# Griffan/FASTQuick

Hardware: AMD Instinct MI355X
Metric: paired_150bp_reads_aligned_per_sec (higher is better)
Workload: dtype u32

## Files before the change

### fastquick_amd/csrc/fq_align.cpp

```cpp
#include <algorithm>
#include <atomic>
#include <ctime>
#include <chrono>
#include <climits>
#include <cstdint>
#include <cmath>
#include <cstdio>
#include <cstdlib>
#include <cstring>
#include <memory>
#include <string>
#include <unordered_map>
#include <mutex>
#include <thread>
#include <vector>
#include <pthread.h>
#include <sched.h>

#include "../../include/fastquick_amd.h"
#include "fq_backend.h"
#include "fq_index.h"
#include "fq_pipeline.h"
#include "fq_pool.h"
#include "fq_text_batch.h"
// ... 368 lines not shown
  else if (k == "gap_long_always") c->kn.gap_long_always = (int)v;
  else if (k == "gap_pool") c->kn.gap_pool = (uint32_t)v;
  else if (k == "gap_nogap_min") c->kn.gap_nogap_min = v;
  else if (k == "gap_pipeline_min") c->kn.gap_pipeline_min = v;
  else if (k == "gap_pipeline_segs") c->kn.gap_pipeline_segs = (int)std::max<int64_t>(2, std::min<int64_t>(v, 64));
  else if (k == "gap_split_hard") c->kn.gap_split_hard = v;
  else if (k == "gap_long_pops2") c->kn.gap_long_pops2 = (uint32_t)v;
  else if (k == "gap_skip_bound") c->kn.gap_skip_bound = v;
  else if (k == "gap_no_order") c->kn.gap_no_order = (int)v;
  else if (k == "device_turns") c->kn.device_turns = (int)v;
  else if (k == "device_turn_min") c->kn.device_turn_min = v;
  else if (k == "device_turn_slots") c->kn.device_turn_slots = (int)std::max<int64_t>(1, v);
  else if (k == "gap_round2_waves") c->kn.gap_round2_waves = (int)v;
  else if (k == "gap_round2_lane_major") c->kn.gap_round2_lane_major = (int)v;
  else if (k == "gap_round1_refill") c->kn.gap_round1_refill = (int)v;
  else if (k == "gap_round2_refill") c->kn.gap_round2_refill = (int)v;
  else if (k == "sw_wave_max") c->kn.sw_wave_max = (int)v;
  else if (k == "host_threads") c->kn.host_threads = (int)v;
  else if (k == "host_par_min") c->kn.host_par_min = (size_t)v;
  else if (k == "packed_bulk_min") c->kn.packed_bulk_min = v;
  else if (k == "md_mask_min") c->kn.md_mask_min = v;
  else if (k == "trace") c->kn.trace = (int)v;
  else if (k == "gap_order_asc") t->gap_order_asc = (int)v;
  else if (k == "gap_waves_per_cu") t->gap_waves_per_cu = (int)v;
  else if (k == "gap_coop_waves") t->gap_coop_waves = (int)v;
  else if (k == "gap_refill_min") t->gap_refill_min = (int)v;
  else if (k == "filter_no_turns") t->filter_no_turns = (int)v;
  else if (k == "prep_priority") t->prep_priority = (int)v;
  else if (k == "refine_lanes") t->refine_lanes = (int)v;
  else if (k == "gap_generic_opts") t->gap_generic_opts = (int)v;
  else if (k == "sw_serial_reverse") t->sw_serial_reverse = (int)v;
  else if (k == "width_both_strands") t->width_both_strands = (int)v;
  else if (k == "spin_sync") t->spin_sync = (int)v;
  else return FQ_EINVAL;
  return FQ_OK;
}

extern "C" void fq_stats_get(const fq_ctx_t *c, fq_stats_t *out) { if (c && out) *out = c->stats; }
extern "C" void fq_stats_reset(fq_ctx_t *c) { if (c) memset(&c->stats, 0, sizeof c->stats); }

#define CK(expr)                                                  \
  do {                                                            \
    if ((expr)) { c->err = std::string(#expr) + ": " + fqdev::last_error(); return FQ_ENODEV; } \
  } while (0)
#define CKM(expr)                                                 \
  do {                                                            \
    if (!(expr)) { c->err = std::string("out of device memory: ") + #expr; return FQ_ENOMEM; } \
  } while (0)

static int h2d_staged(fq_ctx *c, void *dst, const void *src, size_t bytes) {
  if (!bytes) return 0;
  void *p = c->arena.alloc(bytes);
  if (!p) { c->err = "out of pinned host memory"; return FQ_ENOMEM; }
  memcpy(p, src, bytes);
  if (fqdev::copy_pinned(dst, p, bytes, 1)) { c->err = std::string("h2d: ") + fqdev::last_error(); return FQ_ENODEV; }
  return 0;
}
static int d2h_staged(fq_ctx *c, void *dst, const void *src, size_t bytes) {
  if (!bytes) return 0;
  void *p = c->arena.alloc(bytes);
  if (!p) { c->err = "out of pinned host memory"; return FQ_ENOMEM; }
  if (fqdev::copy_pinned(p, src, bytes, 0)) { c->err = std::string("d2h: ") + fqdev::last_error(); return FQ_ENODEV; }
  c->arena.pending.push_back({dst, p, bytes});
  return 0;
}
static int sync_staged(fq_ctx *c) {
// ... 2027 lines not shown
```

### fastquick_amd/csrc/fq_backend.h

```cpp
#pragma once
#include "fq_kernels.h"
#include "fq_records.h"
#include "fq_frontend.h"
#include "fq_emit.h"
#include "fq_deflate.h"

namespace fqdev {

struct State;
struct Tune {
  int gap_coop_waves = 0;
  int gap_waves_per_cu = 0, gap_refill_min = 0, gap_order_asc = 0, filter_no_turns = 0, refine_lanes = 0;
  int spin_sync = 0;
  int gap_generic_opts = 0;
  int width_both_strands = 0;
  int prep_priority = 0;
  int sw_serial_reverse = 0;
};
int runtime_configure(int hw_queues, int blocking_waits);
int device_count();
State *state_create(int device_ordinal);
void state_destroy(State *s);
int bind(State *s);
Tune *tune(State *s);
const char *last_error();
bool is_real_gpu();
void device_turn_begin(int slots = 1);
void device_turn_end();

void *dmalloc(size_t bytes);
void dfree(void *p);
void *hmalloc(size_t bytes);
void hfree(void *p);
int h2d(void *dst, const void *src, size_t bytes);
int d2h(void *dst, const void *src, size_t bytes);
int copy_pinned(void *dst, const void *src, size_t bytes, int to_device);
int d2d(void *dst, const void *src, size_t bytes);
int dzero(void *dst, size_t bytes);
int dfill(void *dst, int byte, size_t bytes);
int sync();
int h2d_copy(void *dst, const void *src, size_t bytes);
int copy_record(int slot);
int copy_wait(int slot);
void copy_discard();
int compute_wait_copy(int slot);
int copy_flush_now();

void time_begin(int kid);
void time_end(int kid);
// ... 52 lines not shown
```

### fastquick_amd/csrc/fq_device.hip

```cpp
#include <hip/hip_runtime.h>
#include <hip/hip_ext.h>

#include <algorithm>
#include <condition_variable>
#include <atomic>
#include <cstdio>
#include <cstdlib>
#include <cstring>
#include <mutex>
#include <string>
#include <unordered_map>
#include <vector>
#include <sys/mman.h>
#include <sys/syscall.h>
#include <unistd.h>

#include "fq_backend.h"

namespace fqdev {

struct Pending { int kid; hipEvent_t a, b; };
struct State {
  int device = 0;
  hipStream_t stream = nullptr;
  hipStream_t main_stream = nullptr, aux_stream = nullptr;
  hipEvent_t fork_ev = nullptr, join_ev = nullptr;
  hipEvent_t marks[4] = {nullptr, nullptr, nullptr, nullptr};
  hipEvent_t prio_fork = nullptr;
  hipStream_t copy_stream = nullptr;
  hipEvent_t copy_done[2] = {nullptr, nullptr};
  hipEvent_t prep_done = nullptr;
  hipEvent_t sync_ev = nullptr;
  std::vector<Pending> pending;
  std::vector<hipEvent_t> free_events;
  hipEvent_t open_begin[16] = {};
  struct SmallCopy { uint8_t *dst; const uint8_t *src; size_t bytes; };
  SmallCopy small[8];
  int n_small = 0;
  uint64_t *scan_tmp = nullptr; size_t scan_tmp_n = 0;
  uint32_t *cmp_cnt = nullptr; uint64_t *cmp_off = nullptr; size_t cmp_n = 0;
  Tune tune;
};
static thread_local State *g_cur = nullptr;
static thread_local std::string g_err;
#define g_stream (g_cur->stream)

#define FQ_HIP(call)                                                                         \
  do {                                                                                       \
    hipError_t e_ = (call);                                                                  \
    if (e_ != hipSuccess) {                                                                  \
      g_err = std::string(#call) + ": " + hipGetErrorString(e_);                             \
      return -3;                                                                             \
    }                                                                                        \
  } while (0)

int copy_flush();
#define FQ_PRE() do { if (copy_flush()) return -3; } while (0)
void copy_discard() { if (g_cur) g_cur->n_small = 0; }
int copy_flush_now() { FQ_PRE(); return 0; }

const char *last_error() { return g_err.c_str(); }
bool is_real_gpu() { return true; }

static int set_kernel_attributes();
static std::mutex g_dev_mu;
static bool g_dev_ready[64];
static hipEvent_t g_prep_last[64];
static State *g_prep_owner[64];
static hipStream_t g_copy_streams[64][2];
static unsigned g_copy_next[64];
static std::mutex g_turn_mu[64];
static std::condition_variable g_turn_cv[64];
static int g_turn_held[64];
static int g_ctx_count[64];
static hipStream_t g_prio_stream[64];
static bool g_queue_warned = false;
static int g_rt_blocking_waits = 0;
int runtime_configure(int hw_queues, int blocking_waits) {
  if (hw_queues > 0) {
    char b[16];
    snprintf(b, sizeof b, "%d", hw_queues);
    setenv("GPU_MAX_HW_QUEUES", b, 0);
  }
  g_rt_blocking_waits = blocking_waits ? 1 : 0;
  return 0;
}

int device_count() { int n = 0; if (hipGetDeviceCount(&n) != hipSuccess) { (void)hipGetLastError(); return 0; } return n < 0 ? 0 : n; }
void device_turn_begin(int slots) {
  const int d = g_cur->device;
  std::unique_lock<std::mutex> lk(g_turn_mu[d]);
// ... 48 lines not shown
  if (s->fork_ev) (void)hipEventDestroy(s->fork_ev);
  if (s->join_ev) (void)hipEventDestroy(s->join_ev);
  for (hipEvent_t m : s->marks) if (m) (void)hipEventDestroy(m);
  if (s->prio_fork) (void)hipEventDestroy(s->prio_fork);
  if (s->stream) (void)hipStreamSynchronize(s->stream);
  if (s->copy_stream) (void)hipStreamSynchronize(s->copy_stream);
  {
    std::lock_guard<std::mutex> lk(g_dev_mu);
    if (g_prep_owner[s->device] == s) { g_prep_owner[s->device] = nullptr; g_prep_last[s->device] = nullptr; }
    if (g_ctx_count[s->device] > 0) --g_ctx_count[s->device];
  }
  for (auto &p : s->pending) { (void)hipEventDestroy(p.a); (void)hipEventDestroy(p.b); }
  for (auto e : s->free_events) (void)hipEventDestroy(e);
  for (auto e : s->copy_done) if (e) (void)hipEventDestroy(e);
  if (s->prep_done) (void)hipEventDestroy(s->prep_done);
  if (s->scan_tmp) (void)hipFree(s->scan_tmp);
  if (s->cmp_cnt) (void)hipFree(s->cmp_cnt);
  if (s->cmp_off) (void)hipFree(s->cmp_off);
  if (s->stream) (void)hipStreamDestroy(s->stream);
  delete s;
}
Tune *tune(State *s) { return &s->tune; }
int bind(State *s) {
  if (!s) { g_err = "no device state"; return -3; }
  if (g_cur != s) { FQ_HIP(hipSetDevice(s->device)); g_cur = s; }
  return 0;
}

void *dmalloc(size_t bytes) {
  void *p = nullptr;
  if (hipMalloc(&p, bytes ? bytes : 16) != hipSuccess) { g_err = "hipMalloc failed (" + std::to_string(bytes) + " B)"; return nullptr; }
  return p;
}
void dfree(void *p) { if (p) (void)hipFree(p); }
static const size_t kRegisterMin = (size_t)4 << 20;
static std::mutex g_reg_mu;
static std::unordered_map<void *, size_t> g_registered;
static int device_numa_node(int dev) {
  static std::mutex mu;
  static std::unordered_map<int, int> cache;
  std::lock_guard<std::mutex> lk(mu);
  auto it = cache.find(dev);
  if (it != cache.end()) return it->second;
  int node = -1;
  char bus[64] = {0};
  if (hipDeviceGetPCIBusId(bus, (int)sizeof bus, dev) == hipSuccess) {
    for (char *c = bus; *c; ++c) if (*c >= 'A' && *c <= 'F') *c = (char)(*c - 'A' + 'a');
    const std::string path = std::string("/sys/bus/pci/devices/") + bus + "/numa_node";
    if (FILE *f = fopen(path.c_str(), "r")) { if (fscanf(f, "%d", &node) != 1) node = -1; fclose(f); }
  } else (void)hipGetLastError();
  cache[dev] = node;
  return node;
}
static void prefer_node(void *m, size_t len, int node) {
  if (node < 0 || node >= 1024) return;
  unsigned long mask[16] = {0};
  mask[node / (8 * sizeof(unsigned long))] |= 1ul << (node % (8 * sizeof(unsigned long)));
  (void)syscall(SYS_mbind, m, len, 1 , mask, (unsigned long)(8 * sizeof mask + 1), 0u);
}
void *hmalloc(size_t bytes) {
  static const bool use_register = [] { const char *e = getenv("FASTQUICK_PIN_REGISTER"); return !(e && *e == '0'); }();
  if (use_register && bytes >= kRegisterMin) {
    const size_t len = (bytes + ((size_t)2 << 20) - 1) & ~(((size_t)2 << 20) - 1);
    void *m = mmap(nullptr, len, PROT_READ | PROT_WRITE, MAP_PRIVATE | MAP_ANONYMOUS, -1, 0);
    if (m != MAP_FAILED) {
      (void)madvise(m, len, MADV_HUGEPAGE);
      int dev = 0;
      if (hipGetDevice(&dev) == hipSuccess) prefer_node(m, len, device_numa_node(dev)); else (void)hipGetLastError();
      if (hipHostRegister(m, len, hipHostRegisterDefault) == hipSuccess) {
        std::lock_guard<std::mutex> lk(g_reg_mu);
        g_registered[m] = len;
        return m;
      }
      (void)hipGetLastError();
      munmap(m, len);
    }
  }
  void *p = nullptr;
  if (hipHostMalloc(&p, bytes ? bytes : 16, hipHostMallocDefault) != hipSuccess) { g_err = "hipHostMalloc failed"; return nullptr; }
  return p;
}
void hfree(void *p) {
  if (!p) return;
  size_t len = 0;
  {
    std::lock_guard<std::mutex> lk(g_reg_mu);
    auto it = g_registered.find(p);
    if (it != g_registered.end()) { len = it->second; g_registered.erase(it); }
  }
  if (len) { (void)hipHostUnregister(p); munmap(p, len); }
  else (void)hipHostFree(p);
}
int h2d(void *dst, const void *src, size_t bytes) { FQ_PRE(); if (bytes) FQ_HIP(hipMemcpyAsync(dst, src, bytes, hipMemcpyHostToDevice, g_stream)); return 0; }
int d2h(void *dst, const void *src, size_t bytes) { FQ_PRE(); if (bytes) FQ_HIP(hipMemcpyAsync(dst, src, bytes, hipMemcpyDeviceToHost, g_stream)); return 0; }
int d2d(void *dst, const void *src, size_t bytes) { FQ_PRE(); if (bytes) FQ_HIP(hipMemcpyAsync(dst, src, bytes, hipMemcpyDeviceToDevice, g_stream)); return 0; }
int dzero(void *dst, size_t bytes) { FQ_PRE(); if (bytes) FQ_HIP(hipMemsetAsync(dst, 0, bytes, g_stream)); return 0; }
int dfill(void *dst, int byte, size_t bytes) { FQ_PRE(); if (bytes) FQ_HIP(hipMemsetAsync(dst, byte, bytes, g_stream)); return 0; }
int sync() {
  FQ_PRE();
  if (g_cur->tune.spin_sync || !g_cur->sync_ev) { FQ_HIP(hipStreamSynchronize(g_stream)); return 0; }
  FQ_HIP(hipEventRecord(g_cur->sync_ev, g_stream));
  FQ_HIP(hipEventSynchronize(g_cur->sync_ev));
  return 0;
}
int stream_aux(int on) {
  FQ_PRE();
  if (on && !g_cur->aux_stream) {
    FQ_HIP(hipStreamCreateWithFlags(&g_cur->aux_stream, hipStreamNonBlocking));
    FQ_HIP(hipEventCreateWithFlags(&g_cur->fork_ev, hipEventDisableTiming));
    FQ_HIP(hipEventCreateWithFlags(&g_cur->join_ev, hipEventDisableTiming));
  }
  g_cur->stream = on ? g_cur->aux_stream : g_cur->main_stream;
  return 0;
}
int stream_fork() {
  FQ_PRE();
  if (!g_cur->aux_stream) return 0;
  FQ_HIP(hipEventRecord(g_cur->fork_ev, g_cur->main_stream));
  FQ_HIP(hipStreamWaitEvent(g_cur->aux_stream, g_cur->fork_ev, 0));
  return 0;
}
int stream_join() {
  FQ_PRE();
  if (!g_cur->aux_stream) return 0;
  FQ_HIP(hipEventRecord(g_cur->join_ev, g_cur->aux_stream));
  FQ_HIP(hipStreamWaitEvent(g_cur->main_stream, g_cur->join_ev, 0));
  return 0;
}
int stream_mark(int k) {
  FQ_PRE();
  hipEvent_t &m = g_cur->marks[k & 3];
  if (!m) FQ_HIP(hipEventCreateWithFlags(&m, hipEventDisableTiming));
  FQ_HIP(hipEventRecord(m, g_stream));
  return 0;
}
int stream_wait_mark(int k) {
  FQ_PRE();
  hipEvent_t m = g_cur->marks[k & 3];
  if (m) FQ_HIP(hipStreamWaitEvent(g_stream, m, 0));
  return 0;
}
static int copy_stream_get() {
  if (g_cur->copy_stream) return 0;
  std::lock_guard<std::mutex> lk(g_dev_mu);
  const int dev = g_cur->device;
  for (int k = 0; k < 2; ++k)
    if (!g_copy_streams[dev][k]) FQ_HIP(hipStreamCreateWithFlags(&g_copy_streams[dev][k], hipStreamNonBlocking));
  g_cur->copy_stream = g_copy_streams[dev][g_copy_next[dev]++ & 1];
  return 0;
}
int h2d_copy(void *dst, const void *src, size_t bytes) {
  if (copy_stream_get()) return -3;
  if (bytes) FQ_HIP(hipMemcpyAsync(dst, src, bytes, hipMemcpyHostToDevice, g_cur->copy_stream));
  return 0;
}
int copy_record(int slot) { if (copy_stream_get()) return -3; FQ_HIP(hipEventRecord(g_cur->copy_done[slot & 1], g_cur->copy_stream)); return 0; }
int copy_wait(int slot) { FQ_HIP(hipEventSynchronize(g_cur->copy_done[slot & 1])); return 0; }
int compute_wait_copy(int slot) { FQ_PRE(); FQ_HIP(hipStreamWaitEvent(g_stream, g_cur->copy_done[slot & 1], 0)); return 0; }

struct FqCopySet { uint8_t *dst[8]; const uint8_t *src[8]; size_t bytes[8]; };
__global__ void __launch_bounds__(256) k_copy_bytes(FqCopySet cs) {
  uint8_t *dst = cs.dst[blockIdx.y];
  const uint8_t *src = cs.src[blockIdx.y];
  const size_t bytes = cs.bytes[blockIdx.y];
  const size_t n16 = ((((uintptr_t)dst | (uintptr_t)src) & 15) == 0) ? bytes / 16 : 0;
  const size_t t = (size_t)blockIdx.x * blockDim.x + threadIdx.x, stride = (size_t)gridDim.x * blockDim.x;
  for (size_t i = t; i < n16; i += stride) ((uint4 *)dst)[i] = ((const uint4 *)src)[i];
  for (size_t i = n16 * 16 + t; i < bytes; i += stride) dst[i] = src[i];
}
static const size_t kSmallCopy = (size_t)8 << 20;
int copy_flush() {
  State *s = g_cur;
  if (!s || s->n_small == 0) return 0;
  FqCopySet cs;
  size_t most = 0;
  for (int k = 0; k < 8; ++k) {
    const bool on = k < s->n_small;
    cs.dst[k] = on ? s->small[k].dst : nullptr; cs.src[k] = on ? s->small[k].src : nullptr; cs.bytes[k] = on ? s->small[k].bytes : 0;
    if (on) most = std::max(most, s->small[k].bytes);
  }
  const int n = s->n_small;
  s->n_small = 0;
  const unsigned blocks = (unsigned)std::min<size_t>(256, (most / 16 + 255) / 256 + 1);
  hipLaunchKernelGGL(k_copy_bytes, dim3(blocks, (unsigned)n), dim3(256), 0, s->stream, cs);
  FQ_HIP(hipGetLastError());
  return 0;
}
int copy_pinned(void *dst, const void *src, size_t bytes, int to_device) {
  if (!bytes) return 0;
  if (bytes > kSmallCopy) { FQ_PRE(); FQ_HIP(hipMemcpyAsync(dst, src, bytes, to_device ? hipMemcpyHostToDevice : hipMemcpyDeviceToHost, g_stream)); return 0; }
  if (g_cur->n_small == 8) FQ_PRE();
  g_cur->small[g_cur->n_small++] = {(uint8_t *)dst, (const uint8_t *)src, bytes};
  return 0;
}

static hipEvent_t get_event() {
  if (!g_cur->free_events.empty()) { hipEvent_t e = g_cur->free_events.back(); g_cur->free_events.pop_back(); return e; }
  hipEvent_t e;
  (void)hipEventCreate(&e);
  return e;
}
void time_begin(int kid) { (void)copy_flush(); hipEvent_t e = get_event(); (void)hipEventRecord(e, g_stream); g_cur->open_begin[kid] = e; }
void time_end(int kid) { (void)copy_flush(); hipEvent_t e = get_event(); (void)hipEventRecord(e, g_stream); g_cur->pending.push_back({kid, g_cur->open_begin[kid], e}); }
static void kernel_events(int kid, hipEvent_t *a, hipEvent_t *b) { *a = get_event(); *b = get_event(); g_cur->pending.push_back({kid, *a, *b}); }
void time_collect(double ms[], uint64_t launches[], int n_ids) {
  std::vector<decltype(g_cur->pending)::value_type> later;
  for (auto &p : g_cur->pending) {
    if (hipEventQuery(p.b) == hipErrorNotReady) { later.push_back(p); continue; }
    float t = 0.f;
    if (hipEventElapsedTime(&t, p.a, p.b) == hipSuccess && p.kid < n_ids) { ms[p.kid] += t; launches[p.kid] += 1; }
    g_cur->free_events.push_back(p.a);
    g_cur->free_events.push_back(p.b);
  }
  g_cur->pending.swap(later);
}

static inline unsigned nblk(uint64_t n, unsigned b) { return (unsigned)((n + b - 1) / b); }

__global__ void __launch_bounds__(256) k_prep(FqPrepArgs a) {
  const int r = blockIdx.x * blockDim.x + threadIdx.x;
  if (r < a.n_reads) fq_prep_thread(a, r);
}
extern __shared__ __align__(16) unsigned char fq_dyn_lds[];
__global__ void __launch_bounds__(256) k_width(FqWidthArgs a) {
  uint8_t *seed_bits = (uint8_t *)fq_dyn_lds;
  const int w = blockIdx.x * blockDim.x + threadIdx.x;
// ... 356 lines not shown
  for (uint32_t base = 0; base < nb; base += 256) {
    const uint32_t i = base + threadIdx.x;
    const uint64_t v = i < nb ? blk_tot[i] : 0;
    const int lane = threadIdx.x & 63, wid = threadIdx.x >> 6;
    __shared__ uint64_t ws[4];
    uint64_t x = v;
#pragma unroll
    for (int d = 1; d < 64; d <<= 1) {
      const uint64_t y = __shfl_up(x, d, 64);
      if (lane >= d) x += y;
    }
    if (lane == 63) ws[wid] = x;
    __syncthreads();
    uint64_t b = carry, tot = 0;
    for (int k = 0; k < 4; ++k) { if (k < wid) b += ws[k]; tot += ws[k]; }
    if (i < nb) blk_tot[i] = b + x - v;
    __syncthreads();
    if (threadIdx.x == 0) carry += tot;
    __syncthreads();
  }
  if (threadIdx.x == 0) blk_tot[nb] = carry;
}
__global__ void __launch_bounds__(256) k_scan_c(const uint32_t *in, uint32_t n, const uint64_t *blk_off, uint64_t *out) {
  const uint32_t i = blockIdx.x * 256 + threadIdx.x;
  uint32_t tot;
  const uint32_t e = block_excl_scan(i < n ? in[i] : 0u, &tot);
  if (i < n) out[i] = blk_off[blockIdx.x] + e;
  if (i == 0) out[n] = blk_off[gridDim.x];
}

#define g_scan_tmp (g_cur->scan_tmp)
#define g_scan_tmp_n (g_cur->scan_tmp_n)
int launch_scan(const uint32_t *in, uint64_t *out, uint32_t n) {
  FQ_PRE();
  if (n == 0) { uint64_t z = 0; return h2d(out, &z, 8) ? -3 : sync(); }
  const unsigned nb = nblk(n, 256);
  if (g_scan_tmp_n < nb + 1) {
    dfree(g_scan_tmp);
    g_scan_tmp_n = (size_t)nb * 2 + 64;
    g_scan_tmp = (uint64_t *)dmalloc(g_scan_tmp_n * 8);
    if (!g_scan_tmp) return -4;
  }
  hipLaunchKernelGGL(k_scan_a, dim3(nb), dim3(256), 0, g_stream, in, n, g_scan_tmp);
  hipLaunchKernelGGL(k_scan_b, dim3(1), dim3(256), 0, g_stream, g_scan_tmp, nb);
  hipLaunchKernelGGL(k_scan_c, dim3(nb), dim3(256), 0, g_stream, in, n, g_scan_tmp, out);
  FQ_HIP(hipGetLastError());
  return 0;
}

__global__ void __launch_bounds__(256) k_compact_a(const uint8_t *filt, int n_pairs, uint32_t *pair_cnt, uint32_t *read_cnt) {
  const int p = blockIdx.x * 256 + threadIdx.x;
  uint32_t keep = 0, nr = 0;
  if (p < n_pairs) {
    const uint32_t f0 = filt[p], f1 = filt[n_pairs + p];
    keep = !(f0 && f1);
    nr = (!f0) + (!f1);
  }
  const unsigned long long bal = __ballot(keep);
  __shared__ uint32_t s_pairs[4], s_reads[4];
  uint32_t x = nr;
#pragma unroll
  for (int d = 32; d >= 1; d >>= 1) x += __shfl_xor(x, d, 64);
  if ((threadIdx.x & 63) == 0) { s_pairs[threadIdx.x >> 6] = (uint32_t)__popcll(bal); s_reads[threadIdx.x >> 6] = x; }
  __syncthreads();
  if (threadIdx.x == 0) {
    pair_cnt[blockIdx.x] = s_pairs[0] + s_pairs[1] + s_pairs[2] + s_pairs[3];
// ... 8 lines not shown
  const uint32_t nr = (!f0) + (!f1);
  uint32_t tot_p, tot_r;
  const uint32_t rank_p = block_excl_scan(keep, &tot_p);
  const uint32_t rank_r = block_excl_scan(nr, &tot_r);
  if (p < n_pairs) {
    if (keep) pair_list[pair_off[blockIdx.x] + rank_p] = p;
    uint32_t s = (uint32_t)read_off[blockIdx.x] + rank_r;
    if (!f0) { read_list[s] = p; sidx[p] = (int32_t)s; ++s; } else sidx[p] = -1;
    if (!f1) { read_list[s] = n_pairs + p; sidx[n_pairs + p] = (int32_t)s; } else sidx[n_pairs + p] = -1;
  }
  if (p == 0) { counts[0] = (int32_t)read_off[gridDim.x]; counts[1] = (int32_t)pair_off[gridDim.x]; }
}
#define g_cmp_cnt (g_cur->cmp_cnt)
#define g_cmp_off (g_cur->cmp_off)
#define g_cmp_n (g_cur->cmp_n)
int launch_compact(const uint8_t *filtered, int n_pairs, int32_t *read_list, int32_t *sidx, int32_t *pair_list, int32_t *counts) {
  FQ_PRE();
  if (n_pairs <= 0) return dzero(counts, 8);
  const unsigned nb = nblk((uint64_t)n_pairs, 256);
  if (g_cmp_n < nb) {
    dfree(g_cmp_cnt); dfree(g_cmp_off);
    g_cmp_n = (size_t)nb * 2 + 64;
    g_cmp_cnt = (uint32_t *)dmalloc(g_cmp_n * 2 * 4);
    g_cmp_off = (uint64_t *)dmalloc((g_cmp_n + 2) * 2 * 8);
    if (!g_cmp_cnt || !g_cmp_off) return -4;
  }
  uint32_t *pc = g_cmp_cnt, *rc = g_cmp_cnt + g_cmp_n;
  uint64_t *po = g_cmp_off, *ro = g_cmp_off + g_cmp_n + 2;
  hipLaunchKernelGGL(k_compact_a, dim3(nb), dim3(256), 0, g_stream, filtered, n_pairs, pc, rc);
  int rc1 = launch_scan(pc, po, nb);
  if (rc1) return rc1;
  rc1 = launch_scan(rc, ro, nb);
  if (rc1) return rc1;
  hipLaunchKernelGGL(k_compact_c, dim3(nb), dim3(256), 0, g_stream, filtered, n_pairs, po, ro, read_list, sidx, pair_list, counts);
  FQ_HIP(hipGetLastError());
  return 0;
}

__global__ void __launch_bounds__(256) k_bitmap_scatter(uint8_t *bitmap, const uint32_t *bits, uint64_t n) {
  const uint64_t i = (uint64_t)blockIdx.x * blockDim.x + threadIdx.x;
  if (i >= n) return;
  const uint32_t x = bits[i];
  atomicOr((unsigned int *)(bitmap + ((x >> 5) << 2)), 1u << (x & 31));
}
int launch_bitmap_scatter(uint8_t *bitmap, const uint32_t *bits, uint64_t n) {
  FQ_PRE();
  if (!n) return 0;
  hipLaunchKernelGGL(k_bitmap_scatter, dim3(nblk(n, 256)), dim3(256), 0, g_stream, bitmap, bits, n);
  FQ_HIP(hipGetLastError());
  return 0;
}

__global__ void __launch_bounds__(256) k_bitmap_kmers(FqBitmapArgs a) {
  const int64_t idx = (int64_t)blockIdx.x * 256 + threadIdx.x;
  if (idx >= 2 * a.l_pac) return;
  fq_bitmap_kmer_thread(a, idx, [&](int t, uint32_t x) { atomicOr(&a.bitmap[t][x >> 5], 1u << (x & 31)); });
}
int launch_bitmap_kmers(const FqBitmapArgs &a) {
  FQ_PRE();
  if (a.l_pac <= 0 || a.n_rec <= 0) return 0;
  hipLaunchKernelGGL(k_bitmap_kmers, dim3(nblk((uint64_t)(2 * a.l_pac), 256)), dim3(256), 0, g_stream, a);
  FQ_HIP(hipGetLastError());
  return 0;
}

static FqzCrcConst *g_crc_const[64];
// ... 65 lines not shown
  const int lane = threadIdx.x & 63;
#pragma unroll
  for (int d = 1; d < 64; d <<= 1) { const uint32_t y = (uint32_t)__shfl_up((int)x, d, 64); if (lane >= d) x += y; }
  __shared__ uint32_t s[4];
  if (lane == 63) s[threadIdx.x >> 6] = x;
  __syncthreads();
  uint32_t base = 0;
  for (int w = 0; w < (int)(threadIdx.x >> 6); ++w) base += s[w];
  uint64_t rank = blk_off[blockIdx.x] + base + (x - c);
  while (m) {
    const int j = __ffs((int)m) - 1;
    m &= m - 1;
    if (rank < cap) nl[rank] = at + (uint32_t)j;
    ++rank;
  }
}
__global__ void __launch_bounds__(64) k_nl_total(const uint64_t *blk_off, uint32_t nb, uint32_t *count) {
  if (threadIdx.x == 0) { const uint64_t t = blk_off[nb]; *count = t > 0xffffffffull ? 0xffffffffu : (uint32_t)t; }
}
int launch_nl_index(const uint8_t *text, uint32_t n, uint32_t lo, uint32_t *nl, uint32_t cap, uint32_t *count) {
  FQ_PRE();
  const unsigned nb = nblk((uint64_t)n, 4096);
  if (nb == 0) { FQ_HIP(hipMemsetAsync(count, 0, 4, g_stream)); return 0; }
  if (g_cmp_n < (size_t)nb + 1) {
    dfree(g_cmp_cnt); dfree(g_cmp_off);
    g_cmp_n = (size_t)nb * 2 + 64;
    g_cmp_cnt = (uint32_t *)dmalloc(g_cmp_n * 2 * 4);
    g_cmp_off = (uint64_t *)dmalloc((g_cmp_n + 2) * 2 * 8);
    if (!g_cmp_cnt || !g_cmp_off) { g_cmp_n = 0; return -4; }
  }
  hipLaunchKernelGGL(k_nl_count, dim3(nb), dim3(256), 0, g_stream, text, n, lo, g_cmp_cnt);
  FQ_HIP(hipGetLastError());
  if (launch_scan(g_cmp_cnt, g_cmp_off, nb)) return -3;
  hipLaunchKernelGGL(k_nl_fill, dim3(nb), dim3(256), 0, g_stream, text, n, lo, (const uint64_t *)g_cmp_off, nl, cap);
  hipLaunchKernelGGL(k_nl_total, dim3(1), dim3(64), 0, g_stream, (const uint64_t *)g_cmp_off, nb, count);
  FQ_HIP(hipGetLastError());
  return 0;
}
__global__ void __launch_bounds__(256) k_tok_rec(FqTokArgs a) {
  const int i = blockIdx.x * 256 + threadIdx.x;
  FqTokStat t = i < a.n_rec ? fqt_rec_thread(a, i) : fqt_stat_none();
#pragma unroll
  for (int d = 32; d >= 1; d >>= 1) {
    t.first_bad = min(t.first_bad, (uint32_t)__shfl_xor((int)t.first_bad, d, 64));
    t.max_name = max(t.max_name, (uint32_t)__shfl_xor((int)t.max_name, d, 64));
    t.min_name = min(t.min_name, (uint32_t)__shfl_xor((int)t.min_name, d, 64));
    t.max_len = max(t.max_len, (uint32_t)__shfl_xor((int)t.max_len, d, 64));
    t.min_len = min(t.min_len, (uint32_t)__shfl_xor((int)t.min_len, d, 64));
  }
  if ((threadIdx.x & 63) == 0) fqt_stat_commit(a, t);
}
__global__ void __launch_bounds__(256) k_tok_pieces(FqTokArgs a, int64_t n) {
  const int64_t g = (int64_t)blockIdx.x * 256 + threadIdx.x;
  if (g < n) fqt_piece_thread(a, g);
}
__global__ void __launch_bounds__(256) k_slot_bases(FqSlotArgs a) {
  const int s = blockIdx.x * 256 + threadIdx.x;
  if (s < a.n_slots) fqt_slot_bases_thread(a, s);
}
__global__ void __launch_bounds__(256) k_slot_names(FqSlotArgs a) {
  const int s = blockIdx.x * 256 + threadIdx.x;
  if (s < a.n_slots) fqt_slot_names_thread(a, s);
}
__global__ void __launch_bounds__(256) k_text_gather(FqTextGatherArgs a, int64_t n) {
  const int64_t g = (int64_t)blockIdx.x * 256 + threadIdx.x;
  if (g < n) fqt_gather_piece(a, g);
// ... 24 lines not shown
  FQ_HIP(hipGetLastError());
  return 0;
}
__global__ void __launch_bounds__(256) k_names_plain(FqSlotArgs a) {
  const int i = blockIdx.x * 256 + threadIdx.x;
  if (i < a.n_rec) fqt_names_plain_thread(a, i);
}
int launch_slot_names(const FqSlotArgs &a) {
  FQ_PRE();
  if (a.n_rec <= 0) return 0;
  if (a.plain_names) {
    hipLaunchKernelGGL(k_names_plain, dim3(nblk((uint64_t)a.n_rec, 256)), dim3(256), 0, g_stream, a);
    if (a.mode != 0) { FQ_HIP(hipGetLastError()); return 0; }
  }
  hipLaunchKernelGGL(k_slot_names, dim3(nblk((uint64_t)a.n_slots, 256)), dim3(256), 0, g_stream, a);
  FQ_HIP(hipGetLastError());
  return 0;
}
int launch_text_gather(const FqTextGatherArgs &a) {
  FQ_PRE();
  const int64_t n = (int64_t)a.n_out * (a.stride >> 4);
  if (n <= 0) return 0;
  hipLaunchKernelGGL(k_text_gather, dim3(nblk((uint64_t)n, 256)), dim3(256), 0, g_stream, a, n);
  FQ_HIP(hipGetLastError());
  return 0;
}
int launch_text_trim_all(const FqTextTrimArgs &a) {
  FQ_PRE();
  if (a.n_rows <= 0) return 0;
  hipLaunchKernelGGL(k_text_trim_all, dim3(nblk((uint64_t)a.n_rows, 256)), dim3(256), 0, g_stream, a);
  FQ_HIP(hipGetLastError());
  return 0;
}
int dfill32(void *dst, uint32_t v, size_t n_words) { FQ_PRE(); if (n_words) FQ_HIP(hipMemsetD32Async((hipDeviceptr_t)dst, (int)v, n_words, g_stream)); return 0; }

int launch_prep(const FqPrepArgs &a) {
  FQ_PRE();
  if (a.n_reads <= 0) return 0;
  hipEvent_t e0, e1;
  kernel_events(FQ_K_PREP_KERNEL, &e0, &e1);
  if (!g_cur->tune.filter_no_turns) {
    const int dev = g_cur->device;
    std::lock_guard<std::mutex> lk(g_dev_mu);
    if (g_prep_last[dev] && g_prep_owner[dev] != g_cur) FQ_HIP(hipStreamWaitEvent(g_stream, g_prep_last[dev], 0));
    hipExtLaunchKernelGGL(k_prep, dim3(nblk((uint64_t)a.n_reads, 256)), dim3(256), 0, g_stream, e0, e1, 0, a);
    FQ_HIP(hipEventRecord(g_cur->prep_done, g_stream));
    g_prep_last[dev] = g_cur->prep_done; g_prep_owner[dev] = g_cur;
  } else {
    hipExtLaunchKernelGGL(k_prep, dim3(nblk((uint64_t)a.n_reads, 256)), dim3(256), 0, g_stream, e0, e1, 0, a);
  }
  FQ_HIP(hipGetLastError());
  return 0;
}
__global__ void __launch_bounds__(256) k_surv_gather(const int32_t *pair_list, int n_surv, int n_pairs, const int32_t *len_trim, const uint8_t *filtered, const int32_t *sidx, FqSurvInfo *out) {
  const int t = blockIdx.x * blockDim.x + threadIdx.x;
  if (t < 2 * n_surv) fq_surv_gather_thread(pair_list, n_pairs, len_trim, filtered, sidx, out, t);
}
int launch_surv_gather(const int32_t *pair_list, int n_surv, int n_pairs, const int32_t *len_trim, const uint8_t *filtered, const int32_t *sidx, FqSurvInfo *out) {
  FQ_PRE();
  if (n_surv <= 0) return 0;
  hipLaunchKernelGGL(k_surv_gather, dim3(nblk((uint64_t)n_surv * 2, 256)), dim3(256), 0, g_stream, pair_list, n_surv, n_pairs, len_trim, filtered, sidx, out);
  FQ_HIP(hipGetLastError());
  return 0;
}
__global__ void __launch_bounds__(256) k_prep_packed(FqPrepPackedArgs a) {
  const int r = blockIdx.x * blockDim.x + threadIdx.x;
  if (r < a.n_reads) fq_prep_packed_thread(a, r);
// ... 131 lines not shown
    base[threadIdx.x] = h[threadIdx.x] ? start + atomicAdd(&cnt[FQ_ORDER_KEYS + threadIdx.x], h[threadIdx.x]) : 0u;
  }
  __syncthreads();
  if (w < n) order[base[key] + rank] = w;
  if (blockIdx.x == 0 && threadIdx.x == 0) {
    uint32_t sp = 0;
    if (asc) { for (int k = 0; k < FQ_ORDER_KEYS / 2; ++k) sp += cnt[k]; }
    else { for (int k = FQ_ORDER_KEYS / 2; k < FQ_ORDER_KEYS; ++k) sp += cnt[k]; }
    cnt[2 * FQ_ORDER_KEYS] = sp;
  }
}
__global__ void __launch_bounds__(256) k_collect(const int32_t *order, const uint32_t *split, int n_work, int seg, int n_seg, const uint32_t *status, const int32_t *work,
                                                  int32_t *out, uint32_t *count) {
  const uint32_t sp = split ? *split : (uint32_t)n_work;
  const uint32_t blk_start[2] = {0u, sp}, blk_len[2] = {sp, (uint32_t)n_work - sp};
  const uint32_t t = blockIdx.x * blockDim.x + threadIdx.x, stride = gridDim.x * blockDim.x;
  for (int b = 0; b < 2; ++b) {
    uint32_t lo, hi;
    fq_seg_range(blk_len[b], seg, n_seg, &lo, &hi);
    for (uint32_t pos = blk_start[b] + lo + t; pos < blk_start[b] + hi; pos += stride) {
      const int w = order ? order[pos] : (int)pos;
      if (status[w]) out[atomicAdd(count, 1u)] = work[w];
    }
  }
}
int launch_collect(const int32_t *order, const uint32_t *split, int n_work, int seg, int n_seg, const uint32_t *status, const int32_t *work, int32_t *out, uint32_t *count) {
  FQ_PRE();
  if (n_work <= 0) return 0;
  hipLaunchKernelGGL(k_collect, dim3(1024), dim3(256), 0, g_stream, order, split, n_work, seg, n_seg, status, work, out, count);
  FQ_HIP(hipGetLastError());
  return 0;
}
int launch_order(const uint8_t *bid_end, int n, int n_hard, int32_t *order, uint32_t *cnt) {
  FQ_PRE();
  if (n <= 0) return 0;
  FQ_HIP(hipMemsetAsync(cnt, 0, (2 * FQ_ORDER_KEYS + 1) * 4, g_stream));
  hipLaunchKernelGGL(k_order_count, dim3(nblk((uint64_t)n, 256)), dim3(256), 0, g_stream, bid_end, n, n_hard, cnt);
  hipLaunchKernelGGL(k_order_scatter, dim3(nblk((uint64_t)n, 256)), dim3(256), 0, g_stream, bid_end, n, n_hard, cnt, order, g_cur->tune.gap_order_asc ? 1 : 0);
  FQ_HIP(hipGetLastError());
  return 0;
}
int gap_lane_slots(const FqGapArgs &a) {
  if (a.n_work <= 0) return 0;
  if (a.tier.coop) {
    const unsigned cw = g_cur->tune.gap_coop_waves > 0 ? (unsigned)g_cur->tune.gap_coop_waves : 1024u;
    unsigned w = std::min<unsigned>((unsigned)a.n_work, a.tier.exact ? 64u : cw);
    if (a.max_waves > 0) w = std::min<unsigned>(w, (unsigned)a.max_waves);
    return (int)w;
  }
  const int env_waves = g_cur->tune.gap_waves_per_cu;
  const unsigned need = nblk((uint64_t)a.n_work, 64);
  unsigned per_cu = 8;
  if (a.tier.pool_cap <= 65535u) {
    const size_t lds = (size_t)64 * (size_t)a.o.n_buckets * 2 + (size_t)64 * FQ_COLD_N * 4;
    per_cu = (unsigned)std::max<size_t>(1, std::min<size_t>(a.tier.nogap ? FQ_NOGAP_WAVES_PER_CU : 16, (150 * 1024) / lds));
  }
  if (env_waves > 0) per_cu = std::min<unsigned>(per_cu, (unsigned)env_waves);
  unsigned waves = std::min(need, 256u * per_cu);
  if (a.max_waves > 0) waves = std::min<unsigned>(waves, (unsigned)a.max_waves);
  return (int)(waves * 64u);
}
int launch_gap(const FqGapArgs &a_in) {
  FQ_PRE();
  if (a_in.n_work <= 0) return 0;
  FqGapArgs a = a_in;
  const int env_refill = g_cur->tune.gap_refill_min;
  a.refill_min = env_refill > 0 ? env_refill : a_in.refill_min > 0 ? a_in.refill_min : FQ_REFILL_MIN;
  FQ_HIP(hipMemsetAsync(a.queue, 0, 8, g_stream));
  hipEvent_t e0, e1;
  kernel_events(a.tier.nogap ? FQ_K_GAP_NOGAP : FQ_K_GAP_KERNEL, &e0, &e1);
  if (a.tier.coop) {
    hipExtLaunchKernelGGL(k_gap_coop, dim3((unsigned)gap_lane_slots(a)), dim3(64), 0, g_stream, e0, e1, 0, a);
  } else {
    const size_t lds = (size_t)64 * (size_t)a.o.n_buckets * 2 + (size_t)64 * FQ_COLD_N * 4;
    const unsigned grid = (unsigned)gap_lane_slots(a) / 64u;
    if (a.tier.exact) { g_err = "launch_gap: the exact tier is the wavefront kernel's"; return -1; }
    const bool stock = FqOptsStock::matches(a.o) && !g_cur->tune.gap_generic_opts;
    if (a.tier.pool_cap <= 65535u && a.tier.nogap) hipExtLaunchKernelGGL(stock ? k_gap_nogap_stock : k_gap_nogap_lds, dim3(grid), dim3(64), lds, g_stream, e0, e1, 0, a);
    else if (a.tier.pool_cap <= 65535u) hipExtLaunchKernelGGL(stock ? k_gap_persist_stock : k_gap_persist_lds, dim3(grid), dim3(64), lds, g_stream, e0, e1, 0, a);
    else hipExtLaunchKernelGGL(k_gap_persist, dim3(grid), dim3(64), 0, g_stream, e0, e1, 0, a);
  }
  FQ_HIP(hipGetLastError());
  return 0;
}
int launch_pack_aln(const FqAln *aln, const uint32_t *n_aln, const uint64_t *off, uint32_t cap, uint32_t n_work, FqAln *packed) {
  FQ_PRE();
  if (!n_work) return 0;
  hipLaunchKernelGGL(k_pack_aln, dim3(nblk(n_work, 256)), dim3(256), 0, g_stream, aln, n_aln, off, cap, n_work, packed);
  FQ_HIP(hipGetLastError());
  return 0;
}
int launch_sa(const FqSaArgs &a) {
  FQ_PRE();
  if (!a.n_rows) return 0;
  hipEvent_t e0, e1;
  kernel_events(FQ_K_SA_KERNEL, &e0, &e1);
  hipExtLaunchKernelGGL(k_sa, dim3(nblk(a.n_rows, 256)), dim3(256), 0, g_stream, e0, e1, 0, a);
  FQ_HIP(hipGetLastError());
  return 0;
}
static const size_t kLdsBudget = 150 * 1024;
// ... 260 lines not shown
```

Baseline: 760.5 million.

## Batch small fills and scans into deferred fused kernels with dependency tracking

Small memsets and fills are queued into the existing deferred small-copy batch, which now also handles fill ops via a fill mode in the copy kernel. Small prefix scans (up to a tunable size) are deferred into a single-block scan kernel that can also write a mirrored slice, which absorbs a following small copy of the scan output. Range-overlap checks flush pending ops only when a real dependency exists. The goal is fewer launches and API calls per batch, at the cost of more host bookkeeping and a serial single-block scan that could be slower for larger inputs.

Result: no change. 762.2 million, median of 4 (+0.2%).

```diff
diff --git a/fastquick_amd/csrc/fq_align.cpp b/fastquick_amd/csrc/fq_align.cpp
--- a/fastquick_amd/csrc/fq_align.cpp
+++ b/fastquick_amd/csrc/fq_align.cpp
@@ -424,6 +424,7 @@
   else if (k == "sw_serial_reverse") t->sw_serial_reverse = (int)v;
   else if (k == "width_both_strands") t->width_both_strands = (int)v;
   else if (k == "spin_sync") t->spin_sync = (int)v;
+  else if (k == "scan_single_max") t->scan_single_max = (int)std::max<int64_t>(0, std::min<int64_t>(v, 65536));
   else return FQ_EINVAL;
   return FQ_OK;
 }
diff --git a/fastquick_amd/csrc/fq_backend.h b/fastquick_amd/csrc/fq_backend.h
--- a/fastquick_amd/csrc/fq_backend.h
+++ b/fastquick_amd/csrc/fq_backend.h
@@ -15,6 +15,7 @@
   int gap_generic_opts = 0;
   int width_both_strands = 0;
   int prep_priority = 0;
+  int scan_single_max = 65536;
   int sw_serial_reverse = 0;
 };
 int runtime_configure(int hw_queues, int blocking_waits);
diff --git a/fastquick_amd/csrc/fq_device.hip b/fastquick_amd/csrc/fq_device.hip
--- a/fastquick_amd/csrc/fq_device.hip
+++ b/fastquick_amd/csrc/fq_device.hip
@@ -34,9 +34,12 @@
   std::vector<Pending> pending;
   std::vector<hipEvent_t> free_events;
   hipEvent_t open_begin[16] = {};
-  struct SmallCopy { uint8_t *dst; const uint8_t *src; size_t bytes; };
-  SmallCopy small[8];
+  struct SmallOp { uint8_t *dst; const uint8_t *src; size_t bytes; uint32_t fill; };
+  SmallOp small[16];
   int n_small = 0;
+  struct SmallScan { const uint32_t *in; uint64_t *out; uint32_t n; uint64_t *mirror; uint32_t m_lo, m_n; };
+  SmallScan scans[4];
+  int n_scan = 0;
   uint64_t *scan_tmp = nullptr; size_t scan_tmp_n = 0;
   uint32_t *cmp_cnt = nullptr; uint64_t *cmp_off = nullptr; size_t cmp_n = 0;
   Tune tune;
@@ -54,9 +57,9 @@
     }                                                                                        \
   } while (0)
 
-int copy_flush();
+int copy_flush(int kinds = 3);
 #define FQ_PRE() do { if (copy_flush()) return -3; } while (0)
-void copy_discard() { if (g_cur) g_cur->n_small = 0; }
+void copy_discard() { if (g_cur) g_cur->n_small = g_cur->n_scan = 0; }
 int copy_flush_now() { FQ_PRE(); return 0; }
 
 const char *last_error() { return g_err.c_str(); }
@@ -171,7 +174,7 @@
   if (hipMalloc(&p, bytes ? bytes : 16) != hipSuccess) { g_err = "hipMalloc failed (" + std::to_string(bytes) + " B)"; return nullptr; }
   return p;
 }
-void dfree(void *p) { if (p) (void)hipFree(p); }
+void dfree(void *p) { if (p) { (void)copy_flush(); (void)hipFree(p); } }
 static const size_t kRegisterMin = (size_t)4 << 20;
 static std::mutex g_reg_mu;
 static std::unordered_map<void *, size_t> g_registered;
@@ -233,8 +236,8 @@
 int h2d(void *dst, const void *src, size_t bytes) { FQ_PRE(); if (bytes) FQ_HIP(hipMemcpyAsync(dst, src, bytes, hipMemcpyHostToDevice, g_stream)); return 0; }
 int d2h(void *dst, const void *src, size_t bytes) { FQ_PRE(); if (bytes) FQ_HIP(hipMemcpyAsync(dst, src, bytes, hipMemcpyDeviceToHost, g_stream)); return 0; }
 int d2d(void *dst, const void *src, size_t bytes) { FQ_PRE(); if (bytes) FQ_HIP(hipMemcpyAsync(dst, src, bytes, hipMemcpyDeviceToDevice, g_stream)); return 0; }
-int dzero(void *dst, size_t bytes) { FQ_PRE(); if (bytes) FQ_HIP(hipMemsetAsync(dst, 0, bytes, g_stream)); return 0; }
-int dfill(void *dst, int byte, size_t bytes) { FQ_PRE(); if (bytes) FQ_HIP(hipMemsetAsync(dst, byte, bytes, g_stream)); return 0; }
+int dfill(void *dst, int byte, size_t bytes);
+int dzero(void *dst, size_t bytes) { return dfill(dst, 0, bytes); }
 int sync() {
   FQ_PRE();
   if (g_cur->tune.spin_sync || !g_cur->sync_ev) { FQ_HIP(hipStreamSynchronize(g_stream)); return 0; }
@@ -297,40 +300,146 @@
 int copy_wait(int slot) { FQ_HIP(hipEventSynchronize(g_cur->copy_done[slot & 1])); return 0; }
 int compute_wait_copy(int slot) { FQ_PRE(); FQ_HIP(hipStreamWaitEvent(g_stream, g_cur->copy_done[slot & 1], 0)); return 0; }
 
-struct FqCopySet { uint8_t *dst[8]; const uint8_t *src[8]; size_t bytes[8]; };
+struct FqCopySet { uint8_t *dst[16]; const uint8_t *src[16]; size_t bytes[16]; uint32_t fill[16]; };
 __global__ void __launch_bounds__(256) k_copy_bytes(FqCopySet cs) {
   uint8_t *dst = cs.dst[blockIdx.y];
   const uint8_t *src = cs.src[blockIdx.y];
   const size_t bytes = cs.bytes[blockIdx.y];
+  const size_t t = (size_t)blockIdx.x * blockDim.x + threadIdx.x, stride = (size_t)gridDim.x * blockDim.x;
+  if (!src) {
+    const uint32_t v = cs.fill[blockIdx.y];
+    const size_t lead = (size_t)(-(uintptr_t)dst & 15), head = lead < bytes ? lead : bytes, n16 = (bytes - head) / 16;
+    const uint32_t w = head & 3 ? (v >> (8 * (head & 3))) | (v << (32 - 8 * (head & 3))) : v;
+    const uint4 w4 = make_uint4(w, w, w, w);
+    for (size_t i = t; i < n16; i += stride) ((uint4 *)(dst + head))[i] = w4;
+    for (size_t i = t; i < head; i += stride) dst[i] = (uint8_t)(v >> (8 * (i & 3)));
+    for (size_t i = head + n16 * 16 + t; i < bytes; i += stride) dst[i] = (uint8_t)(v >> (8 * (i & 3)));
+    return;
+  }
   const size_t n16 = ((((uintptr_t)dst | (uintptr_t)src) & 15) == 0) ? bytes / 16 : 0;
-  const size_t t = (size_t)blockIdx.x * blockDim.x + threadIdx.x, stride = (size_t)gridDim.x * blockDim.x;
   for (size_t i = t; i < n16; i += stride) ((uint4 *)dst)[i] = ((const uint4 *)src)[i];
   for (size_t i = n16 * 16 + t; i < bytes; i += stride) dst[i] = src[i];
 }
 static const size_t kSmallCopy = (size_t)8 << 20;
-int copy_flush() {
+struct FqScanSet { const uint32_t *in[4]; uint64_t *out[4]; uint64_t *mirror[4]; uint32_t n[4], m_lo[4], m_n[4]; };
+__global__ void __launch_bounds__(1024) k_scan_small(FqScanSet ss) {
+  const uint32_t *in = ss.in[blockIdx.x];
+  uint64_t *out = ss.out[blockIdx.x];
+  const uint32_t n = ss.n[blockIdx.x];
+  uint64_t *mirror = ss.mirror[blockIdx.x];
+  const uint64_t m_lo = ss.m_lo[blockIdx.x], m_hi = mirror ? m_lo + ss.m_n[blockIdx.x] : 0;
+  __shared__ uint64_t ws[16];
+  const int lane = threadIdx.x & 63, wid = threadIdx.x >> 6;
+  uint64_t carry = 0;
+  for (uint64_t base = 0; base < n; base += 4096) {
+    const uint64_t i0 = base + (uint64_t)threadIdx.x * 4;
+    uint32_t v[4];
+#pragma unroll
+    for (int k = 0; k < 4; ++k) v[k] = i0 + k < n ? in[i0 + k] : 0u;
+    const uint64_t s = (uint64_t)v[0] + v[1] + v[2] + v[3];
+    uint64_t x = s;
+#pragma unroll
+    for (int d = 1; d < 64; d <<= 1) {
+      const uint64_t y = __shfl_up(x, d, 64);
+      if (lane >= d) x += y;
+    }
+    if (lane == 63) ws[wid] = x;
+    __syncthreads();
+    uint64_t e = carry + x - s, tot = 0;
+#pragma unroll
+    for (int k = 0; k < 16; ++k) { if (k < wid) e += ws[k]; tot += ws[k]; }
+#pragma unroll
+    for (int k = 0; k < 4; ++k) {
+      if (i0 + k < n) { out[i0 + k] = e; if (i0 + k >= m_lo && i0 + k < m_hi) mirror[i0 + k - m_lo] = e; }
+      e += v[k];
+    }
+    carry += tot;
+    __syncthreads();
+  }
+  if (threadIdx.x == 0) { out[n] = carry; if (n >= m_lo && n < m_hi) mirror[n - m_lo] = carry; }
+}
+int copy_flush(int kinds) {
   State *s = g_cur;
-  if (!s || s->n_small == 0) return 0;
-  FqCopySet cs;
-  size_t most = 0;
-  for (int k = 0; k < 8; ++k) {
-    const bool on = k < s->n_small;
-    cs.dst[k] = on ? s->small[k].dst : nullptr; cs.src[k] = on ? s->small[k].src : nullptr; cs.bytes[k] = on ? s->small[k].bytes : 0;
-    if (on) most = std::max(most, s->small[k].bytes);
-  }
-  const int n = s->n_small;
-  s->n_small = 0;
-  const unsigned blocks = (unsigned)std::min<size_t>(256, (most / 16 + 255) / 256 + 1);
-  hipLaunchKernelGGL(k_copy_bytes, dim3(blocks, (unsigned)n), dim3(256), 0, s->stream, cs);
-  FQ_HIP(hipGetLastError());
+  if (!s || (s->n_small == 0 && s->n_scan == 0)) return 0;
+  if ((kinds & 1) && s->n_small) {
+    FqCopySet cs;
+    size_t most = 0;
+    for (int k = 0; k < 16; ++k) {
+      const bool on = k < s->n_small;
+      cs.dst[k] = on ? s->small[k].dst : nullptr; cs.src[k] = on ? s->small[k].src : nullptr; cs.bytes[k] = on ? s->small[k].bytes : 0; cs.fill[k] = on ? s->small[k].fill : 0;
+      if (on) most = std::max(most, s->small[k].bytes);
+    }
+    const int n = s->n_small;
+    s->n_small = 0;
+    const unsigned blocks = (unsigned)std::min<size_t>(256, (most / 16 + 255) / 256 + 1);
+    hipLaunchKernelGGL(k_copy_bytes, dim3(blocks, (unsigned)n), dim3(256), 0, s->stream, cs);
+  }
+  if ((kinds & 2) && s->n_scan) {
+    FqScanSet ss;
+    for (int k = 0; k < 4; ++k) {
+      const bool on = k < s->n_scan;
+      ss.in[k] = on ? s->scans[k].in : nullptr; ss.out[k] = on ? s->scans[k].out : nullptr; ss.n[k] = on ? s->scans[k].n : 0;
+      ss.mirror[k] = on ? s->scans[k].mirror : nullptr; ss.m_lo[k] = on ? s->scans[k].m_lo : 0; ss.m_n[k] = on ? s->scans[k].m_n : 0;
+    }
+    const int n = s->n_scan;
+    s->n_scan = 0;
+    hipLaunchKernelGGL(k_scan_small, dim3((unsigned)n), dim3(1024), 0, s->stream, ss);
+  }
+  FQ_HIP(hipGetLastError());
+  return 0;
+}
+static inline bool ranges_meet(const void *a, size_t na, const void *b, size_t nb) {
+  return na && nb && (uintptr_t)a < (uintptr_t)b + nb && (uintptr_t)b < (uintptr_t)a + na;
+}
+static int queue_depends(const void *rd, size_t n_rd, const void *wr, size_t n_wr) {
+  const State *s = g_cur;
+  int on = 0;
+  for (int k = 0; k < s->n_small; ++k) {
+    const State::SmallOp &o = s->small[k];
+    if (ranges_meet(wr, n_wr, o.dst, o.bytes) || (o.src && ranges_meet(wr, n_wr, o.src, o.bytes)) || ranges_meet(rd, n_rd, o.dst, o.bytes)) on |= 1;
+  }
+  for (int k = 0; k < s->n_scan; ++k) {
+    const State::SmallScan &o = s->scans[k];
+    const size_t n_out = ((size_t)o.n + 1) * 8, n_mir = o.mirror ? (size_t)o.m_n * 8 : 0;
+    if (ranges_meet(wr, n_wr, o.out, n_out) || ranges_meet(wr, n_wr, o.mirror, n_mir) || ranges_meet(wr, n_wr, o.in, (size_t)o.n * 4) ||
+        ranges_meet(rd, n_rd, o.out, n_out) || ranges_meet(rd, n_rd, o.mirror, n_mir)) on |= 2;
+  }
+  return on;
+}
+static bool scan_mirror(uint8_t *dst, const uint8_t *src, size_t bytes) {
+  State *s = g_cur;
+  if (((uintptr_t)dst | bytes) & 7) return false;
+  for (int k = 0; k < s->n_scan; ++k) {
+    State::SmallScan &o = s->scans[k];
+    const uint8_t *lo = (const uint8_t *)o.out, *hi = lo + ((size_t)o.n + 1) * 8;
+    if (o.mirror || src < lo || src + bytes > hi || ((src - lo) & 7)) continue;
+    if (queue_depends(nullptr, 0, dst, bytes)) return false;
+    o.mirror = (uint64_t *)dst; o.m_lo = (uint32_t)((src - lo) / 8); o.m_n = (uint32_t)(bytes / 8);
+    return true;
+  }
+  return false;
+}
+static int queue_small(uint8_t *dst, const uint8_t *src, size_t bytes, uint32_t fill) {
+  if (src && scan_mirror(dst, src, bytes)) return 0;
+  const int on = queue_depends(src, src ? bytes : 0, dst, bytes) | (g_cur->n_small == 16 ? 1 : 0);
+  if (on && copy_flush(on)) return -3;
+  g_cur->small[g_cur->n_small++] = {dst, src, bytes, fill};
   return 0;
 }
 int copy_pinned(void *dst, const void *src, size_t bytes, int to_device) {
   if (!bytes) return 0;
   if (bytes > kSmallCopy) { FQ_PRE(); FQ_HIP(hipMemcpyAsync(dst, src, bytes, to_device ? hipMemcpyHostToDevice : hipMemcpyDeviceToHost, g_stream)); return 0; }
-  if (g_cur->n_small == 8) FQ_PRE();
-  g_cur->small[g_cur->n_small++] = {(uint8_t *)dst, (const uint8_t *)src, bytes};
-  return 0;
+  return queue_small((uint8_t *)dst, (const uint8_t *)src, bytes, 0);
+}
+int dfill(void *dst, int byte, size_t bytes) {
+  if (!bytes) return 0;
+  if (bytes > kSmallCopy) { FQ_PRE(); FQ_HIP(hipMemsetAsync(dst, byte, bytes, g_stream)); return 0; }
+  return queue_small((uint8_t *)dst, nullptr, bytes, 0x01010101u * (uint32_t)(byte & 0xff));
+}
+int dfill32(void *dst, uint32_t v, size_t n_words) {
+  if (!n_words) return 0;
+  if (n_words * 4 > kSmallCopy || ((uintptr_t)dst & 3)) { FQ_PRE(); FQ_HIP(hipMemsetD32Async((hipDeviceptr_t)dst, (int)v, n_words, g_stream)); return 0; }
+  return queue_small((uint8_t *)dst, nullptr, n_words * 4, v);
 }
 
 static hipEvent_t get_event() {
@@ -753,6 +862,12 @@
 #define g_scan_tmp (g_cur->scan_tmp)
 #define g_scan_tmp_n (g_cur->scan_tmp_n)
 int launch_scan(const uint32_t *in, uint64_t *out, uint32_t n) {
+  if (n && n <= (uint32_t)std::max(0, g_cur->tune.scan_single_max)) {
+    const int on = queue_depends(in, (size_t)n * 4, out, ((size_t)n + 1) * 8) | (g_cur->n_scan == 4 ? 2 : 0);
+    if (on && copy_flush(on)) return -3;
+    g_cur->scans[g_cur->n_scan++] = {in, out, n, nullptr, 0, 0};
+    return 0;
+  }
   FQ_PRE();
   if (n == 0) { uint64_t z = 0; return h2d(out, &z, 8) ? -3 : sync(); }
   const unsigned nb = nblk(n, 256);
@@ -827,6 +942,7 @@
   if (rc1) return rc1;
   rc1 = launch_scan(rc, ro, nb);
   if (rc1) return rc1;
+  FQ_PRE();
   hipLaunchKernelGGL(k_compact_c, dim3(nb), dim3(256), 0, g_stream, filtered, n_pairs, po, ro, read_list, sidx, pair_list, counts);
   FQ_HIP(hipGetLastError());
   return 0;
@@ -958,6 +1074,7 @@
   hipLaunchKernelGGL(k_nl_count, dim3(nb), dim3(256), 0, g_stream, text, n, lo, g_cmp_cnt);
   FQ_HIP(hipGetLastError());
   if (launch_scan(g_cmp_cnt, g_cmp_off, nb)) return -3;
+  FQ_PRE();
   hipLaunchKernelGGL(k_nl_fill, dim3(nb), dim3(256), 0, g_stream, text, n, lo, (const uint64_t *)g_cmp_off, nl, cap);
   hipLaunchKernelGGL(k_nl_total, dim3(1), dim3(64), 0, g_stream, (const uint64_t *)g_cmp_off, nb, count);
   FQ_HIP(hipGetLastError());
@@ -1048,7 +1165,6 @@
   FQ_HIP(hipGetLastError());
   return 0;
 }
-int dfill32(void *dst, uint32_t v, size_t n_words) { FQ_PRE(); if (n_words) FQ_HIP(hipMemsetD32Async((hipDeviceptr_t)dst, (int)v, n_words, g_stream)); return 0; }
 
 int launch_prep(const FqPrepArgs &a) {
   FQ_PRE();
@@ -1246,9 +1362,9 @@
   return 0;
 }
 int launch_order(const uint8_t *bid_end, int n, int n_hard, int32_t *order, uint32_t *cnt) {
-  FQ_PRE();
-  if (n <= 0) return 0;
-  FQ_HIP(hipMemsetAsync(cnt, 0, (2 * FQ_ORDER_KEYS + 1) * 4, g_stream));
+  if (n <= 0) { FQ_PRE(); return 0; }
+  if (dfill32(cnt, 0, 2 * FQ_ORDER_KEYS + 1)) return -3;
+  FQ_PRE();
   hipLaunchKernelGGL(k_order_count, dim3(nblk((uint64_t)n, 256)), dim3(256), 0, g_stream, bid_end, n, n_hard, cnt);
   hipLaunchKernelGGL(k_order_scatter, dim3(nblk((uint64_t)n, 256)), dim3(256), 0, g_stream, bid_end, n, n_hard, cnt, order, g_cur->tune.gap_order_asc ? 1 : 0);
   FQ_HIP(hipGetLastError());
@@ -1275,12 +1391,12 @@
   return (int)(waves * 64u);
 }
 int launch_gap(const FqGapArgs &a_in) {
-  FQ_PRE();
-  if (a_in.n_work <= 0) return 0;
+  if (a_in.n_work <= 0) { FQ_PRE(); return 0; }
+  if (dfill32(a_in.queue, 0, 2)) return -3;
+  FQ_PRE();
   FqGapArgs a = a_in;
   const int env_refill = g_cur->tune.gap_refill_min;
   a.refill_min = env_refill > 0 ? env_refill : a_in.refill_min > 0 ? a_in.refill_min : FQ_REFILL_MIN;
-  FQ_HIP(hipMemsetAsync(a.queue, 0, 8, g_stream));
   hipEvent_t e0, e1;
   kernel_events(a.tier.nogap ? FQ_K_GAP_NOGAP : FQ_K_GAP_KERNEL, &e0, &e1);
   if (a.tier.coop) {
```
